# carlobaldassi/GaussDCA.jl

Measured on AMD Instinct MI355X. Metric: end-to-end gDCA sec + achieved Cholesky TFLOP/s, N=500 M=50k q=21, higher is better.
Workload: dtype f64

## Files before the change

### gaussdca.jl_amd/csrc/gdca_api.hip

```cpp
#include <algorithm>
#include <ctype.h>
#include <math.h>
#include <stdio.h>
#include <stdlib.h>
#include <string.h>
#include <strings.h>

#include "gdca_internal.h"
#include "gdca_launch.h"

#define MAX_EV 1024
#define N_SCRATCH 10

struct gdca_buf {
    void *p;
    size_t cap;
};

struct gdca_gate {
    hipEvent_t ev[4];
    int next, last, armed, refs;
    hipStream_t batch_stream;
};

// ... 246 lines not shown
    if (!strncasecmp(key, "GDCA_", 5)) key += 5;
    for (; key[n] && n + 1 < sizeof(k); ++n) k[n] = (char)toupper((unsigned char)key[n]);
    k[n] = 0;
    if (!strcmp(k, "SWEEP_TRACE")) {
        if (strlen(value) >= sizeof(t->sweep_trace)) return false;
        strcpy(t->sweep_trace, value);
        return true;
    }
    if (!strcmp(k, "HAMMING_MODE")) {
        const char c = (char)tolower((unsigned char)value[0]);
        t->hamming_mode = c == 'f' ? 0 : (c == 'b' ? 1 : (c == 'm' ? 2 : -1));
        return c == 'f' || c == 'b' || c == 'm' || c == 'a' || c == 0;
    }
    if (!strcmp(k, "FORCE_FALLBACK")) {
        t->force_fallback = (*value && strcmp(value, "0") != 0) ? 1 : 0;
        return true;
    }
    long x = 0;
    if (strcmp(k, "REFINE") && strcmp(k, "REFINE_COND") && !parse_long(value, &x)) return false;
    struct { const char *name; int *field; long lo, hi; } ints[] = {
        {"GROUP", &t->group, -1, 4},        {"RAMP", &t->ramp, 0, 1},          {"RAGGED", &t->ragged, 0, 1},
        {"REM_TAIL", &t->rem_tail, -1, 1 << 20}, {"PANEL_HALVES", &t->panel_halves, -1, 1}, {"SLAB", &t->slab, 0, 1},
        {"RING", &t->ring, 2, 8},           {"MCUS", &t->mcus, -1, 32},        {"MCU_SOLO", &t->mcu_solo, -1, 1},       {"SWEEP_DEBUG", &t->sweep_debug, 0, 63}, {"SWEEP_RETRIES", &t->sweep_retries, 0, 5},
        {"TALLY_TJ", &t->tally_tj, 0, 32},  {"TALLY_SKIP", &t->tally_skip, 0, 1}, {"MERGE", &t->merge, 1, 8},        {"MERGE_BLOCKS", &t->merge_blocks, 1, 64},
        {"MERGE_MCUS", &t->merge_mcus, -1, 16},  {"MERGE_GROUP", &t->merge_group, -1, 4}, {"MERGE_TILES", &t->merge_tiles, 1, 1 << 20},
        {"CHOLESKY", &t->cholesky, 0, 2},  {"PHASED_FRONTS", &t->phased_fronts, 0, 1}, {"PHASED_GRIDS", &t->phased_grids, -1, 8}, {"PHASED_STREAMS", &t->phased_streams, 1, 64},
        {"ENERGY_CHUNK", &t->energy_chunk, 0, 1 << 30}, {"PAIR_CHUNK", &t->pair_chunk, 0, 1 << 30},
    };
    for (auto &e : ints)
        if (!strcmp(k, e.name)) {
            if (x < e.lo || x > e.hi) return false;
            *e.field = (int)x;
            return true;
        }
    if (!strcmp(k, "REFINE")) {
        const char c = (char)tolower((unsigned char)value[0]);
        if (c == 'a' || !strcmp(value, "-1")) t->refine = -1;
        else if (!strcmp(value, "0") || !strcasecmp(value, "off") || c == 'n') t->refine = 0;
        else if (!strcmp(value, "1") || !strcasecmp(value, "on") || c == 'y') t->refine = 1;
        else return false;
        return true;
    }
    if (!strcmp(k, "REFINE_COND")) {
        char *end = nullptr;
        const double x = strtod(value, &end);
        if (end == value || *end || !(x > 0.0)) return false;
        t->refine_cond = x;
// ... 1 lines not shown
    }
    if (!strcmp(k, "SWEEP_TIMEOUT_MS")) {
        if (x < 0) return false;
        t->sweep_timeout_ms = x;
        return true;
    }
    return false;
}

void gdca_tuning_from_env(gdca_tuning *t)
{
    memset(t, 0, sizeof(*t));
    t->group = -1;
    t->ramp = 1;
    t->ragged = 1;
    t->rem_tail = -1;
    t->panel_halves = -1;
    t->slab = 1;
    t->ring = 8;
    t->mcus = -1;
    t->mcu_solo = -1;
    t->sweep_retries = 2;
    t->tally_skip = 1;
    t->hamming_mode = -1;
    t->merge = 8;
    t->merge_blocks = 57;
    t->merge_mcus = -1;
    t->merge_group = -1;
    t->merge_tiles = 2300;
    t->phased_fronts = 1;
    t->phased_grids = -1;
    t->phased_streams = 4;
    t->refine = -1;
    t->refine_cond = 1e6;
    t->cholesky = 1;
    static const char *const names[] = {"GDCA_GROUP", "GDCA_RAMP", "GDCA_RAGGED", "GDCA_REM_TAIL", "GDCA_PANEL_HALVES", "GDCA_SLAB",
                                        "GDCA_RING", "GDCA_MCUS", "GDCA_SWEEP_DEBUG", "GDCA_SWEEP_TIMEOUT_MS", "GDCA_SWEEP_RETRIES", "GDCA_TALLY_TJ", "GDCA_TALLY_SKIP",
                                        "GDCA_HAMMING_MODE", "GDCA_FORCE_FALLBACK", "GDCA_MERGE", "GDCA_MERGE_BLOCKS",
                                        "GDCA_MERGE_MCUS", "GDCA_MERGE_GROUP", "GDCA_MERGE_TILES", "GDCA_REFINE", "GDCA_REFINE_COND", "GDCA_CHOLESKY", "GDCA_SWEEP_TRACE", "GDCA_PHASED_FRONTS", "GDCA_PHASED_GRIDS", "GDCA_PHASED_STREAMS", "GDCA_MCU_SOLO", "GDCA_ENERGY_CHUNK", "GDCA_PAIR_CHUNK"};
    for (const char *nm : names)
        if (const char *v = getenv(nm)) (void)gdca_tuning_set(t, nm, v);
}

static gdca_status fail(gdca_ctx *ctx, gdca_status st, const char *fmt, const char *a, const char *b)
{
    if (ctx) snprintf(ctx->err, sizeof(ctx->err), fmt, a, b);
    return st;
}

#define HIPCHK(expr)                                                                      \
    do {                                                                                  \
        hipError_t e_ = (expr);                                                           \
        if (e_ != hipSuccess) return fail(ctx, GDCA_EHIP, "%s: %s", #expr, hipGetErrorString(e_)); \
    } while (0)

#define CHK(expr)                         \
    do {                                  \
        gdca_status s_ = (expr);          \
        if (s_ != GDCA_OK) return s_;     \
    } while (0)

static gdca_status ensure(gdca_ctx *ctx, gdca_buf &b, size_t bytes)
{
    if (bytes == 0) bytes = 16;
    if (b.cap >= bytes) return GDCA_OK;
    if (b.p) {
        HIPCHK(hipStreamSynchronize(ctx->stream));
        HIPCHK(hipFree(b.p));
        b.p = nullptr;
        b.cap = 0;
    }
    const size_t want = (bytes + 255) & ~(size_t)255;
    hipError_t e = hipMalloc(&b.p, want);
// ... 248 lines not shown
        memcpy(lead->err, msg, sizeof(msg));
    }
    return st;
}

static gdca_status upload_done(gdca_ctx *ctx)
{
    HIPCHK(hipEventRecord(ctx->ev_upload, ctx->stream));
    HIPCHK(hipEventSynchronize(ctx->ev_upload));
    return GDCA_OK;
}

static double inverse_flops_model(double n)
{
    return (n * n * n / 3.0 + n * n / 2.0 + n / 6.0) + (2.0 * n * n * n / 3.0 + n * n / 2.0 + 5.0 * n / 6.0);
}

static int round_up(int x, int m)
{
    return (x + m - 1) / m * m;
}

static gdca_status weights_stage(gdca_ctx *ctx, const int8_t *Zd, int N, int M, int q, double theta_in, int fixed_thresh,
                                 bool want_theta_only, int mark_after_theta)
{
    hipStream_t s = ctx->stream;
    gdca_dev_scalars *sc = (gdca_dev_scalars *)ctx->sc.p;
    CHK(ensure(ctx, ctx->hist, (size_t)N * 32 * sizeof(uint32_t)));
    if (fixed_thresh >= 0) {
        gdca_launch_set_thresh(s, sc, fixed_thresh);
    } else {
        if (theta_in < 0.0) {
            gdca_fill_async(s, ctx->hist.p, 0, (size_t)N * 32 * sizeof(uint32_t));
            gdca_launch_column_hist(s, Zd, (uint32_t *)ctx->hist.p, N, M);
        }
        gdca_launch_theta_finalize(s, (const uint32_t *)ctx->hist.p, N, M, theta_in, sc);
    }
    CHK(check_launch(ctx, "theta"));
    if (mark_after_theta >= 0) CHK(mark(ctx, mark_after_theta));
    if (want_theta_only) return GDCA_OK;

    const int Mt = (M + GDCA_HTILE - 1) / GDCA_HTILE;
    CHK(ensure(ctx, ctx->Zb, gdca_bitplane_bytes(N, M)));
    CHK(ensure(ctx, ctx->hcnt, (size_t)Mt * GDCA_HTILE * sizeof(int32_t)));
    if (!ctx->tune.force_fallback && ctx->tune.hamming_mode != 0) CHK(ensure(ctx, ctx->hcand, gdca_hamming_cand_cap(M) * 8));
    const bool fp4 = !ctx->tune.force_fallback && ctx->tune.hamming_mode == 2;
    if (fp4) CHK(ensure(ctx, ctx->himg, gdca_fp4_image_bytes(N, M)));
    CHK(ensure(ctx, ctx->nk, (size_t)M * sizeof(int32_t)));
    CHK(ensure(ctx, ctx->W, (size_t)M * sizeof(double)));
    CHK(ensure(ctx, ctx->Wfix, (size_t)M * sizeof(unsigned long long)));
    gdca_fill_async(s, ctx->hcnt.p, 0, (size_t)Mt * GDCA_HTILE * sizeof(int32_t));
    gdca_launch_bitplane_pack(s, Zd, (uint32_t *)ctx->Zb.p, N, M, q, sc);
    if (ctx->tune.force_fallback)
        gdca_launch_hamming_fallback(s, Zd, (int32_t *)ctx->hcnt.p, N, M, sc);
    else
        gdca_launch_hamming(s, (const uint32_t *)ctx->Zb.p, Zd, (int32_t *)ctx->hcnt.p, N, M, sc, ctx->tune.hamming_mode, ctx->hcand.p, fp4 ? ctx->himg.p : nullptr);
    gdca_launch_weights(s, (const int32_t *)ctx->hcnt.p, M, gdca_fix_shift(M), (int32_t *)ctx->nk.p,
                        (double *)ctx->W.p, (unsigned long long *)ctx->Wfix.p);
    gdca_launch_meff(s, (const double *)ctx->W.p, M, sc);
    return check_launch(ctx, "weights");
}

static bool norm1_settled(const gdca_ctx *ctx, int N, int q, double pc)
{
    const double pi_cap = (1.0 - pc) + pc / (double)q;
    return pc > 0.0 && 2.0 * (double)N * pi_cap * (double)q * (double)q / pc <= ctx->tune.refine_cond && ctx->tune.refine != 1;
}

static gdca_status tally_stage(gdca_ctx *ctx, const int8_t *Zd, int N, int M, int q, const double *Meff_dev, double pc,
                               int mode, double *Pi_true_out, double *out, size_t ld, bool want_norm1 = false)
{
    hipStream_t s = ctx->stream;
    const int sdim = q - 1, n = N * sdim;
    const int shift = gdca_fix_shift(M);
    const int TJ = gdca_tally_tj(q, ctx->tune.tally_tj);
    const bool skip = gdca_tally_skip(q, TJ, ctx->tune.tally_skip, M);
    const size_t keep_list = (size_t)N * M * sizeof(uint32_t);
    if (skip) CHK(ensure(ctx, ctx->keep, keep_list + (size_t)N * sizeof(int) + N));
    CHK(ensure(ctx, ctx->Zt, (size_t)N * M));
    CHK(ensure(ctx, ctx->Zp, (size_t)round_up(N, 64) * M + 64));
    CHK(ensure(ctx, ctx->Pifix, (size_t)N * 32 * sizeof(unsigned long long)));
    CHK(ensure(ctx, ctx->Pipc, (size_t)n * sizeof(double)));
    gdca_launch_transpose_i8(s, Zd, (int8_t *)ctx->Zt.p, N, M);
    gdca_launch_colblock(s, Zd, (int8_t *)ctx->Zp.p, N, M, TJ);
    gdca_fill_async(s, ctx->Pifix.p, 0, (size_t)N * 32 * sizeof(unsigned long long));
    gdca_launch_pi_tally(s, Zd, (const unsigned long long *)ctx->Wfix.p, (unsigned long long *)ctx->Pifix.p, N, M, q,
                         (gdca_dev_scalars *)ctx->sc.p);
    gdca_launch_pi_finalize(s, (const unsigned long long *)ctx->Pifix.p, N, q, shift, Meff_dev, pc, Pi_true_out,
                            (double *)ctx->Pipc.p, want_norm1 ? &((gdca_dev_scalars *)ctx->sc.p)->pi_max : nullptr);
    const bool tm = want_norm1 && ctx->timing && ctx->n_ev >= 18;
    if (tm) CHK(mark(ctx, 9));
    uint32_t *keep = skip ? (uint32_t *)ctx->keep.p : nullptr;
    int *keep_n = skip ? (int *)((char *)ctx->keep.p + keep_list) : nullptr;
    uint8_t *sigma = skip ? (uint8_t *)(keep_n + N) : nullptr;
    if (skip)
        gdca_launch_tally_keep(s, (const int8_t *)ctx->Zt.p, (const unsigned long long *)ctx->Pifix.p, keep, keep_n, sigma, N, M, q);
    gdca_launch_pair_tally(s, (const int8_t *)ctx->Zp.p, (const int8_t *)ctx->Zt.p,
                           (const unsigned long long *)ctx->Wfix.p, N, M, q, shift, Meff_dev, pc,
                           (const double *)ctx->Pipc.p, mode, out, ld, TJ, keep, keep_n, sigma,
                           (const unsigned long long *)ctx->Pifix.p);
    if (tm) CHK(mark(ctx, 10));
    if (want_norm1 && !norm1_settled(ctx, N, q, pc))
        gdca_launch_cov_norm1(s, out, ld, N, q, pc, ctx->tune.refine_cond, (gdca_dev_scalars *)ctx->sc.p, ctx->tune.refine == 1);
    return check_launch(ctx, "tally");
}

static gdca_status inverse_job(gdca_ctx *ctx, int n, int n_pad, gdca_inverse_job *job)
{
    const size_t pbytes = (size_t)n_pad * GDCA_TILE * sizeof(double);
    const int nblk = n_pad / GDCA_TILE;
    const size_t sg = (size_t)4 * GDCA_TILE * 4 * GDCA_TILE * sizeof(double);
    const size_t fbytes = gdca_inverse_flag_bytes(n_pad);
    CHK(ensure(ctx, ctx->G, (size_t)8 * pbytes));
    CHK(ensure(ctx, ctx->H, (size_t)8 * pbytes));
    CHK(ensure(ctx, ctx->P, (size_t)GDCA_TILE * GDCA_TILE * sizeof(double)));
    CHK(ensure(ctx, ctx->Sg, 4 * sg + fbytes + (size_t)3 * (nblk + 2) * sizeof(int)));
    if (ctx->item0_cap < 3 * (nblk + 2)) {
        if (ctx->item0_host) HIPCHK(hipHostFree(ctx->item0_host));
// ... 408 lines not shown
    r.q = q;
    r.n = N * (q - 1);
    r.n_pad = round_up(r.n, GDCA_TILE);
    r.Z = Z_dev;
    r.pij = pij;
    r.p = *p;
    r.timed = timed;
    r.stamped = ctx->stamped;
    r.front_batch = r.score_batch = 1;
    r.tally_timed = timed && !pij && ctx->tune.refine != 0;
    r.fn_timed = false;
}

static gdca_status run_front(gdca_ctx *ctx, const int8_t *Z_dev, int32_t N, int32_t M, int32_t q, const gdca_params *p)
{
    CHK(begin(ctx));
    hipStream_t s = ctx->stream;
    const int sdim = q - 1, n = N * sdim, n_pad = round_up(n, GDCA_TILE);
    const bool timed = ctx->timing;
    if (timed) CHK(need_events(ctx, 18));
    gdca_dev_scalars *sc = (gdca_dev_scalars *)ctx->sc.p;

    if (timed) CHK(mark(ctx, 0));
    CHK(weights_stage(ctx, Z_dev, N, M, q, p->theta, -1, false, timed ? 1 : -1));
    if (timed) CHK(mark(ctx, 2));

    CHK(ensure(ctx, ctx->A, (size_t)n_pad * n_pad * sizeof(double)));
    CHK(tally_stage(ctx, Z_dev, N, M, q, &sc->Meff, p->pseudocount, 1, nullptr, (double *)ctx->A.p, (size_t)n_pad, ctx->tune.refine != 0));
    gdca_launch_pad_identity(s, (double *)ctx->A.p, n, n_pad);
    if (p->score == GDCA_SCORE_DI) {
        CHK(ensure(ctx, ctx->Dblk, (size_t)N * sdim * sdim * sizeof(double)));
        CHK(ensure(ctx, ctx->Ld, (size_t)N * sdim * sdim * sizeof(double)));
        gdca_launch_save_diag_blocks(s, (const double *)ctx->A.p, (size_t)n_pad, N, sdim, (double *)ctx->Dblk.p);
        gdca_launch_diag_chol(s, (const double *)ctx->Dblk.p, N, sdim, (double *)ctx->Ld.p);
    }
    CHK(check_launch(ctx, "covariance"));
    if (timed) CHK(mark(ctx, 3));
    pending_front(ctx, Z_dev, N, M, q, p, nullptr, timed);
    return GDCA_OK;
}

static gdca_status run_inverse(gdca_ctx *ctx)
{
    hipStream_t s = ctx->stream;
    const bool timed = ctx->pend.timed;
    hipEvent_t *ev = ctx->ev;
    int n_upd = 0;
    double upd_flops = 0.0;
    if (ctx->gate) HIPCHK(gate_wait(ctx->gate, s));
    if (timed) HIPCHK(hipEventRecord(ev[6], s));
    CHK(inverse_stage(ctx, ctx->pend.n, ctx->pend.n_pad, timed, &n_upd, &upd_flops));
// ... 477 lines not shown
    double *sv;
    CHK(ranking_stage(ctx, S_dev, ctx->pend.N, rk->sep, rk->len, &ii, &jj, &sv));
    const size_t at = (size_t)k * (size_t)rk->len;
    return ranking_to_host(ctx, rk->len, ii, jj, sv, rk->i_out + at, rk->j_out + at, rk->score_out + at);
}

static gdca_status run_multi(gdca_ctx *ctx, const int8_t *Z_dev, int N, int M, int q, const gdca_params *p, int K, double *S_dev, size_t S_stride,
                             gdca_stats *st, const multi_rank *rk)
{
    hipStream_t s = ctx->stream;
    const int sdim = q - 1, n = N * sdim, n_pad = round_up(n, GDCA_TILE);
    gdca_status mst[GDCA_MULTI_MAX];
    bool done[GDCA_MULTI_MAX];
    for (int k = 0; k < K; ++k) {
        memset(&st[k], 0, sizeof(st[k]));
        mst[k] = GDCA_OK;
        done[k] = false;
    }
    CHK(begin(ctx));
    const bool timed = ctx->timing;
    if (timed) CHK(need_events(ctx, 18));
    gdca_dev_scalars *sc = (gdca_dev_scalars *)ctx->sc.p;
    if (timed) CHK(mark(ctx, 0));
    CHK(weights_stage(ctx, Z_dev, N, M, q, p[0].theta, -1, false, timed ? 1 : -1));
    if (timed) CHK(mark(ctx, 2));
    CHK(ensure(ctx, ctx->Pij, (size_t)n * n * sizeof(double)));
    CHK(ensure(ctx, ctx->A, (size_t)n_pad * n_pad * sizeof(double)));
    CHK(ensure(ctx, ctx->sc_front, sizeof(gdca_dev_scalars)));
    CHK(tally_stage(ctx, Z_dev, N, M, q, &sc->Meff, p[0].pseudocount, 0, nullptr, (double *)ctx->Pij.p, (size_t)n));
    HIPCHK(hipMemcpyAsync(ctx->sc_front.p, sc, sizeof(gdca_dev_scalars), hipMemcpyDeviceToDevice, s));
    pending_front(ctx, Z_dev, N, M, q, &p[0], (const double *)ctx->Pij.p, timed);
    double ms_theta = 0.0, ms_weights = 0.0;
    bool first = true;
    for (int k0 = 0; k0 < K; ++k0) {
        if (done[k0]) continue;
        const double pc = p[k0].pseudocount;
        bool di = false;
        for (int k = k0; k < K; ++k) di = di || (p[k].pseudocount == pc && p[k].score == GDCA_SCORE_DI);
        if (!first) {
            HIPCHK(hipMemcpyAsync(sc, ctx->sc_front.p, sizeof(gdca_dev_scalars), hipMemcpyDeviceToDevice, s));
            ctx->pend.at = gdca_pending::progress{};
            if (timed) CHK(mark(ctx, 2));
        }
        ctx->pend.p = p[k0];
        ctx->pend.fn_timed = false;
        CHK(cov_from_pij_stage(ctx, N, M, q, pc, (double *)ctx->A.p, (size_t)n_pad, ctx->tune.refine != 0));
        gdca_launch_pad_identity(s, (double *)ctx->A.p, n, n_pad);
        if (di) {
            CHK(ensure(ctx, ctx->Dblk, (size_t)N * sdim * sdim * sizeof(double)));
            CHK(ensure(ctx, ctx->Ld, (size_t)N * sdim * sdim * sizeof(double)));
            gdca_launch_save_diag_blocks(s, (const double *)ctx->A.p, (size_t)n_pad, N, sdim, (double *)ctx->Dblk.p);
            gdca_launch_diag_chol(s, (const double *)ctx->Dblk.p, N, sdim, (double *)ctx->Ld.p);
// ... 835 lines not shown
```

### gaussdca.jl_amd/csrc/gdca_internal.h

```cpp
#pragma once

#include <hip/hip_runtime.h>
#include <stdint.h>

#include "gdca.h"

#define GDCA_TILE 128
#define GDCA_HTILE 128
#define GDCA_MAXQ 31
#define GDCA_STAMPS 20

struct gdca_dev_scalars {
    double theta;
    double Meff;
    unsigned long long pair_sum;
    int thresh;
    int info;
    int bad_symbol;
    int di_noconv;
    int ham_mode;
    int ham_cand;
    unsigned long long ham_ncand;
    unsigned long long sweep_cycles, sweep_ticks;
    double inv_norm1;
    double ns_resid;
    double mat_norm1;
    double pi_max;
    unsigned long long stamp[GDCA_STAMPS];
    int ham_cand2;
    int pad_;
};

struct gdca_tuning {
    int group;
    int ramp;
    int ragged;
    int rem_tail;
    int panel_halves;
    int slab;
    int ring;
    int mcus;
    int mcu_solo;
    int sweep_debug;
    long sweep_timeout_ms;
    int sweep_retries;
    int tally_tj;
    int tally_skip;
    int hamming_mode;
    int force_fallback;
    int merge;
    int merge_blocks;
    int merge_mcus;
    int merge_group;
    int merge_tiles;
    int phased_fronts;
    int phased_grids;
    int phased_streams;
    int refine;
    double refine_cond;
    int cholesky;
    int energy_chunk;
    int pair_chunk;
    char sweep_trace[256];
};
void gdca_tuning_from_env(gdca_tuning *t);
bool gdca_tuning_set(gdca_tuning *t, const char *key, const char *value);

void gdca_launch_transpose_i8(hipStream_t s, const int8_t *Z, int8_t *Zt, int N, int M);
void gdca_launch_column_hist(hipStream_t s, const int8_t *Z, uint32_t *cnt, int N, int M);
void gdca_launch_theta_finalize(hipStream_t s, const uint32_t *cnt, int N, int M, double theta_in,
                                gdca_dev_scalars *sc);
void gdca_launch_set_thresh(hipStream_t s, gdca_dev_scalars *sc, int thresh);

size_t gdca_bitplane_bytes(int N, int M);
void gdca_launch_bitplane_pack(hipStream_t s, const int8_t *Z, uint32_t *Zb, int N, int M, int q,
                               gdca_dev_scalars *sc);
size_t gdca_hamming_cand_cap(int M);
size_t gdca_fp4_image_bytes(int N, int M);
void gdca_launch_hamming_fp4_probe(hipStream_t s, const uint32_t *Zb, int N, int M, int nprobe, gdca_dev_scalars *sc);
void gdca_launch_hamming_fp4(hipStream_t s, const uint32_t *Zb, void *img, int N, int M, gdca_dev_scalars *sc, void *cand_list, unsigned cap);
void gdca_launch_hamming(hipStream_t s, const uint32_t *Zb, const int8_t *Z, int32_t *cnt, int N, int M, gdca_dev_scalars *sc, int force,
                         void *cand_list, void *fp4_img);
void gdca_launch_hamming_fallback(hipStream_t s, const int8_t *Z, int32_t *cnt, int N, int M, const gdca_dev_scalars *sc);
void gdca_launch_weights(hipStream_t s, const int32_t *cnt, int M, int fix_shift, int32_t *n_out, double *W,
                         unsigned long long *Wfix);
void gdca_launch_meff(hipStream_t s, const double *W, int M, gdca_dev_scalars *sc);
void gdca_launch_fix_weights(hipStream_t s, const double *W, int M, int fix_shift, unsigned long long *Wfix,
                             gdca_dev_scalars *sc);
int gdca_fix_shift(int M);

void gdca_launch_pi_tally(hipStream_t s, const int8_t *Z, const unsigned long long *Wfix,
                          unsigned long long *Pifix, int N, int M, int q, gdca_dev_scalars *sc);
void gdca_launch_pi_finalize(hipStream_t s, const unsigned long long *Pifix, int N, int q, int fix_shift,
                             const double *Meff_dev, double pc, double *Pi_true, double *Pi_pc, double *pi_max = nullptr);
void gdca_launch_cov_norm1(hipStream_t s, const double *C, size_t ld, int N, int q, double pc, double cond_limit, gdca_dev_scalars *sc,
                           int always);
int gdca_tally_tj(int q, int tj_wanted);
void gdca_launch_colblock(hipStream_t s, const int8_t *Z, int8_t *Zc, int N, int M, int TJ);
bool gdca_tally_skip(int q, int TJ, int skip_wanted, int M);
void gdca_launch_tally_keep(hipStream_t s, const int8_t *Zt, const unsigned long long *Pifix, uint32_t *keep, int *keep_n,
                            uint8_t *sigma, int N, int M, int q);
void gdca_launch_pair_tally(hipStream_t s, const int8_t *Zc, const int8_t *Zt, const unsigned long long *Wfix,
                            int N, int M, int q, int fix_shift, const double *Meff_dev, double pc,
                            const double *Pi_pc, int mode, double *out, size_t ld, int TJ, const uint32_t *keep = nullptr,
                            const int *keep_n = nullptr, const uint8_t *sigma = nullptr, const unsigned long long *Pifix = nullptr);
void gdca_launch_cov_from_pij(hipStream_t s, const double *Pij, const double *Pi_pc, int N, int q, double pc, double *out, size_t ld);

void gdca_launch_add_pseudocount(hipStream_t s, const double *Pi_true, const double *Pij_true, int N, int q,
                                 double pc, double *Pi, double *Pij);
void gdca_launch_covariance(hipStream_t s, const double *Pi, const double *Pij, int n, double *C);
void gdca_launch_pad_identity(hipStream_t s, double *A, int n, int n_pad);
void gdca_launch_copy_in(hipStream_t s, const double *src, int n, double *dst, int n_pad);
void gdca_launch_copy_in_neg(hipStream_t s, const double *src, int n, double *dst, int n_pad);
void gdca_launch_copy_out_neg_sym(hipStream_t s, const double *A, int n_pad, double *dst, int n);
void gdca_launch_publish_scalars(hipStream_t s, const gdca_dev_scalars *sc, gdca_dev_scalars *host_mapped);
void gdca_launch_save_diag_blocks(hipStream_t s, const double *C, size_t ld, int N, int sdim, double *D);

struct gdca_inverse_ws {
    double *G[8];
    double *H[8];
    double *P;
    double *Sg[2];
    double *Pg[2];
    unsigned *flags;
// ... 63 lines not shown
```

### gaussdca.jl_amd/csrc/k_tally.hip

```cpp
#include "gdca_internal.h"
#include "gdca_launch.h"
#include <cstdlib>

typedef unsigned long long u64;

struct k_pi_tally_args {
    const int8_t *Z;
    const u64 *Wfix;
    u64 *Pifix;
    int N;
    int M;
    int seq_per_block;
    int q;
    gdca_dev_scalars *sc;
};
static inline k_pi_tally_args k_pi_tally_mk(const int8_t *Z, const u64 *Wfix, u64 *Pifix, int N, int M, int seq_per_block, int q, gdca_dev_scalars *sc)
{
    return k_pi_tally_args{Z, Wfix, Pifix, N, M, seq_per_block, q, sc};
}
template <int CAP>
__global__ __launch_bounds__(128) void k_pi_tally(const BatchArgs<k_pi_tally_args, CAP> B_)
{
    GDCA_MEMBER(B_);
    const int8_t *__restrict__ Z = a_.Z;
// ... 189 lines not shown
        const int k = k0 + r * 4 + ty, c = c0 + tx;
        tile[r * 4 + ty][tx] = (k < M && c < N) ? Z[(size_t)k * N + c] : (int8_t)0;
    }
    __syncthreads();
    const int nb = 64 / TJ;
    for (int e = threadIdx.x; e < 64 * 64; e += 256) {
        const int blk = e / (64 * TJ), rem = e % (64 * TJ);
        const int kl = rem / TJ, cl = rem % TJ;
        const int k = k0 + kl;
        const int cb = c0 / TJ + blk;
        if (blk < nb && k < M && cb * TJ < ((N + TJ - 1) / TJ) * TJ)
            Zc[((size_t)cb * M + k) * TJ + cl] = tile[kl][blk * TJ + cl];
    }
}

void gdca_launch_colblock(hipStream_t s, const int8_t *Z, int8_t *Zc, int N, int M, int TJ)
{
    dim3 grid((N + 63) / 64, (M + 63) / 64);
    (gdca_launch<k_colblock_args, k_colblock<1>, k_colblock<GDCA_MAXB>>(grid, dim3(256), 0, s, k_colblock_mk(Z, Zc, N, M, TJ)));
}

#define KEEP_THREADS 256
#define KEEP_SLABS 16
struct k_tally_keep_args {
    const int8_t *Zt;
    const u64 *Pifix;
    uint32_t *keep;
    int *keep_n;
    uint8_t *sigma;
    int N;
    int M;
    int q;
};
static inline k_tally_keep_args k_tally_keep_mk(const int8_t *Zt, const u64 *Pifix, uint32_t *keep, int *keep_n, uint8_t *sigma, int N, int M, int q)
{
    return k_tally_keep_args{Zt, Pifix, keep, keep_n, sigma, N, M, q};
}
template <int CAP>
__global__ __launch_bounds__(KEEP_THREADS) void k_tally_keep(const BatchArgs<k_tally_keep_args, CAP> B_)
{
    GDCA_MEMBER(B_);
    const int8_t *__restrict__ Zt = a_.Zt;
    const u64 *__restrict__ Pifix = a_.Pifix;
    uint32_t *__restrict__ keep = a_.keep;
    int M = a_.M;
    int q = a_.q;
    constexpr int NW = KEEP_THREADS / 64;
    __shared__ unsigned wcnt[KEEP_SLABS * NW], woff[KEEP_SLABS * NW];
    const int i = blockIdx.x;
    const int t = threadIdx.x, lane = t & 63, wv = t >> 6;
    const u64 *P = Pifix + (size_t)i * 32;
    unsigned sig = 1;
    u64 best = P[1];
    for (int a = 2; a <= q; ++a) {
        const u64 v = P[a];
        if (v > best) {
            best = v;
            sig = (unsigned)a;
        }
    }
    const int8_t *zi = Zt + (size_t)i * M;
    uint32_t *out = keep + (size_t)i * M;
    const u64 lt = (1ull << lane) - 1ull;
    unsigned base = 0;
    for (int kc = 0; kc < M; kc += KEEP_THREADS * KEEP_SLABS) {
        unsigned raw[KEEP_SLABS], pos[KEEP_SLABS];
#pragma unroll
        for (int u = 0; u < KEEP_SLABS; ++u) {
            const int k = kc + u * KEEP_THREADS + t;
            raw[u] = k < M ? (unsigned)(uint8_t)zi[k] : 0u;
        }
#pragma unroll
        for (int u = 0; u < KEEP_SLABS; ++u) {
            const bool kp = (raw[u] - 1u) < (unsigned)q && raw[u] != sig;
            const u64 bal = __ballot(kp);
            pos[u] = kp ? (unsigned)__popcll(bal & lt) : ~0u;
            if (lane == 0) wcnt[u * NW + wv] = (unsigned)__popcll(bal);
        }
        __syncthreads();
        if (t < KEEP_SLABS * NW) {
            unsigned o = base;
            for (int e = 0; e < t; ++e) o += wcnt[e];
            woff[t] = o;
        }
        __syncthreads();
#pragma unroll
        for (int u = 0; u < KEEP_SLABS; ++u)
            if (pos[u] != ~0u) out[woff[u * NW + wv] + pos[u]] = ((unsigned)(kc + u * KEEP_THREADS + t) << 5) | raw[u];
        base = woff[KEEP_SLABS * NW - 1] + wcnt[KEEP_SLABS * NW - 1];
        __syncthreads();
    }
    if (t == 0) {
        a_.keep_n[i] = (int)base;
        a_.sigma[i] = (uint8_t)sig;
    }
}

void gdca_launch_tally_keep(hipStream_t s, const int8_t *Zt, const u64 *Pifix, uint32_t *keep, int *keep_n, uint8_t *sigma, int N, int M, int q)
{
    (gdca_launch<k_tally_keep_args, k_tally_keep<1>, k_tally_keep<GDCA_MAXB>>(dim3(N), dim3(KEEP_THREADS), 0, s, k_tally_keep_mk(Zt, Pifix, keep, keep_n, sigma, N, M, q)));
}

struct k_pair_tally_args {
    const int8_t *Zc;
    const int8_t *Zt;
    const u64 *Wfix;
    int N;
    int M;
    int q;
    int fix_shift;
    const double *Meff_dev;
    double pc;
    const double *Pi_pc;
    int mode;
    double *out;
    size_t ld;
    const uint32_t *keep;
    const int *keep_n;
    const uint8_t *sigma;
    const u64 *Pifix;
};
static inline k_pair_tally_args k_pair_tally_mk(const int8_t *Zc, const int8_t *Zt, const u64 *Wfix, int N, int M, int q, int fix_shift, const double *Meff_dev, double pc, const double *Pi_pc, int mode, double *out, size_t ld,
                                                const uint32_t *keep, const int *keep_n, const uint8_t *sigma, const u64 *Pifix)
// ... 259 lines not shown
```

### gaussdca.jl_amd/csrc/k_theta.hip

```cpp
#include "gdca_internal.h"
#include "gdca_launch.h"

struct k_transpose_i8_args {
    const int8_t *Z;
    int8_t *Zt;
    int N;
    int M;
};
static inline k_transpose_i8_args k_transpose_i8_mk(const int8_t *Z, int8_t *Zt, int N, int M)
{
    return k_transpose_i8_args{Z, Zt, N, M};
}
template <int CAP>
__global__ __launch_bounds__(256) void k_transpose_i8(const BatchArgs<k_transpose_i8_args, CAP> B_)
{
    GDCA_MEMBER(B_);
    const int8_t *__restrict__ Z = a_.Z;
    int8_t *__restrict__ Zt = a_.Zt;
    int N = a_.N;
    int M = a_.M;
    __shared__ int8_t tile[64][65];
    const int k0 = blockIdx.y * 64, i0 = blockIdx.x * 64;
    const int tx = threadIdx.x & 63, ty = threadIdx.x >> 6;
#pragma unroll
// ... 53 lines not shown
            for (int u = 0; u < 16; ++u) h[z[u]][t] += 1;
            p += (size_t)16 * N;
        }
        for (; k < kend; ++k) {
            h[p[0] & 31][t] += 1;
            p += N;
        }
#pragma unroll
        for (int z = 0; z < 32; ++z) {
            const uint32_t v = h[z][t];
            if (v) atomicAdd(&cnt[(size_t)i * 32 + z], v);
        }
    }
}

void gdca_launch_column_hist(hipStream_t s, const int8_t *Z, uint32_t *cnt, int N, int M)
{
    const int cb = (N + 255) / 256;
    int chunks = (256 + cb - 1) / cb;
    int spb = (M + chunks - 1) / chunks;
    if (spb < 64) spb = 64;
    chunks = (M + spb - 1) / spb;
    (gdca_launch<k_column_hist_args, k_column_hist<1>, k_column_hist<GDCA_MAXB>>(dim3(cb, chunks), dim3(256), 0, s, k_column_hist_mk(Z, cnt, N, M, spb)));
}

struct k_theta_finalize_args {
    const uint32_t *cnt;
    int N;
    int M;
    double theta_in;
    gdca_dev_scalars *sc;
};
static inline k_theta_finalize_args k_theta_finalize_mk(const uint32_t *cnt, int N, int M, double theta_in, gdca_dev_scalars *sc)
{
    return k_theta_finalize_args{cnt, N, M, theta_in, sc};
}
template <int CAP>
__global__ __launch_bounds__(256) void k_theta_finalize(const BatchArgs<k_theta_finalize_args, CAP> B_)
{
    GDCA_MEMBER(B_);
    const uint32_t *__restrict__ cnt = a_.cnt;
    int N = a_.N;
    int M = a_.M;
    double theta_in = a_.theta_in;
    gdca_dev_scalars *sc = a_.sc;
    __shared__ unsigned long long red[256];
// ... 62 lines not shown
```

Measured before the change: 47.36.

## Fuse front-end passes over Z into a single prepare kernel and merge pi tally with keep

Adds a k_prepare kernel that reads the alignment once per tile and in the same pass produces the bitplane pack, the transposed Zt, the column-blocked Zc, the column histogram and the symbol validity check. These were previously separate kernels that each read Z again. Also adds a k_pi_keep kernel that computes the single-site tally from Zt and builds the keep list in the same block, replacing the separate pi_tally and tally_keep launches. Both paths are on by default through a new FRONT_FUSED knob; the cost is a more complex kernel with heavy shared-memory use and possible changes in occupancy.

Result: no change. 47.72 (median of 6 runs) (+0.8%).

```diff
diff --git a/gaussdca.jl_amd/csrc/gdca_api.hip b/gaussdca.jl_amd/csrc/gdca_api.hip
--- a/gaussdca.jl_amd/csrc/gdca_api.hip
+++ b/gaussdca.jl_amd/csrc/gdca_api.hip
@@ -292,7 +292,7 @@
         {"GROUP", &t->group, -1, 4},        {"RAMP", &t->ramp, 0, 1},          {"RAGGED", &t->ragged, 0, 1},
         {"REM_TAIL", &t->rem_tail, -1, 1 << 20}, {"PANEL_HALVES", &t->panel_halves, -1, 1}, {"SLAB", &t->slab, 0, 1},
         {"RING", &t->ring, 2, 8},           {"MCUS", &t->mcus, -1, 32},        {"MCU_SOLO", &t->mcu_solo, -1, 1},       {"SWEEP_DEBUG", &t->sweep_debug, 0, 63}, {"SWEEP_RETRIES", &t->sweep_retries, 0, 5},
-        {"TALLY_TJ", &t->tally_tj, 0, 32},  {"TALLY_SKIP", &t->tally_skip, 0, 1}, {"MERGE", &t->merge, 1, 8},        {"MERGE_BLOCKS", &t->merge_blocks, 1, 64},
+        {"TALLY_TJ", &t->tally_tj, 0, 32},  {"TALLY_SKIP", &t->tally_skip, 0, 1}, {"FRONT_FUSED", &t->front_fused, 0, 1}, {"MERGE", &t->merge, 1, 8},        {"MERGE_BLOCKS", &t->merge_blocks, 1, 64},
         {"MERGE_MCUS", &t->merge_mcus, -1, 16},  {"MERGE_GROUP", &t->merge_group, -1, 4}, {"MERGE_TILES", &t->merge_tiles, 1, 1 << 20},
         {"CHOLESKY", &t->cholesky, 0, 2},  {"PHASED_FRONTS", &t->phased_fronts, 0, 1}, {"PHASED_GRIDS", &t->phased_grids, -1, 8}, {"PHASED_STREAMS", &t->phased_streams, 1, 64},
         {"ENERGY_CHUNK", &t->energy_chunk, 0, 1 << 30}, {"PAIR_CHUNK", &t->pair_chunk, 0, 1 << 30},
@@ -340,6 +340,7 @@
     t->mcu_solo = -1;
     t->sweep_retries = 2;
     t->tally_skip = 1;
+    t->front_fused = 1;
     t->hamming_mode = -1;
     t->merge = 8;
     t->merge_blocks = 57;
@@ -353,7 +354,7 @@
     t->refine_cond = 1e6;
     t->cholesky = 1;
     static const char *const names[] = {"GDCA_GROUP", "GDCA_RAMP", "GDCA_RAGGED", "GDCA_REM_TAIL", "GDCA_PANEL_HALVES", "GDCA_SLAB",
-                                        "GDCA_RING", "GDCA_MCUS", "GDCA_SWEEP_DEBUG", "GDCA_SWEEP_TIMEOUT_MS", "GDCA_SWEEP_RETRIES", "GDCA_TALLY_TJ", "GDCA_TALLY_SKIP",
+                                        "GDCA_RING", "GDCA_MCUS", "GDCA_SWEEP_DEBUG", "GDCA_SWEEP_TIMEOUT_MS", "GDCA_SWEEP_RETRIES", "GDCA_TALLY_TJ", "GDCA_TALLY_SKIP", "GDCA_FRONT_FUSED",
                                         "GDCA_HAMMING_MODE", "GDCA_FORCE_FALLBACK", "GDCA_MERGE", "GDCA_MERGE_BLOCKS",
                                         "GDCA_MERGE_MCUS", "GDCA_MERGE_GROUP", "GDCA_MERGE_TILES", "GDCA_REFINE", "GDCA_REFINE_COND", "GDCA_CHOLESKY", "GDCA_SWEEP_TRACE", "GDCA_PHASED_FRONTS", "GDCA_PHASED_GRIDS", "GDCA_PHASED_STREAMS", "GDCA_MCU_SOLO", "GDCA_ENERGY_CHUNK", "GDCA_PAIR_CHUNK"};
     for (const char *nm : names)
@@ -366,7 +367,12 @@
     return st;
 }
 
-#define HIPCHK(expr)                                                                      \
+static gdca_status fail(gdca_ctx *ctx, gdca_status st, const char *msg)
+{
+    return fail(ctx, st, "%s%s", msg, "");
+}
+
+#define HIPCHK(expr)                                                                     \
     do {                                                                                  \
         hipError_t e_ = (expr);                                                           \
         if (e_ != hipSuccess) return fail(ctx, GDCA_EHIP, "%s: %s", #expr, hipGetErrorString(e_)); \
@@ -661,12 +667,21 @@
 }
 
 static gdca_status weights_stage(gdca_ctx *ctx, const int8_t *Zd, int N, int M, int q, double theta_in, int fixed_thresh,
-                                 bool want_theta_only, int mark_after_theta)
+                                 bool want_theta_only, int mark_after_theta, bool fused = false)
 {
     hipStream_t s = ctx->stream;
     gdca_dev_scalars *sc = (gdca_dev_scalars *)ctx->sc.p;
+    if (fused && (fixed_thresh >= 0 || want_theta_only)) return fail(ctx, GDCA_EINVAL, "weights_stage: the fused form takes theta and runs the whole stage");
     CHK(ensure(ctx, ctx->hist, (size_t)N * 32 * sizeof(uint32_t)));
-    if (fixed_thresh >= 0) {
+    if (fused) {
+        CHK(ensure(ctx, ctx->Zb, gdca_bitplane_bytes(N, M)));
+        CHK(ensure(ctx, ctx->Zt, (size_t)N * M));
+        CHK(ensure(ctx, ctx->Zp, (size_t)round_up(N, 64) * M + 64));
+        if (theta_in < 0.0) gdca_fill_async(s, ctx->hist.p, 0, (size_t)N * 32 * sizeof(uint32_t));
+        gdca_launch_prepare(s, Zd, (uint32_t *)ctx->Zb.p, (int8_t *)ctx->Zt.p, (int8_t *)ctx->Zp.p, theta_in < 0.0 ? (uint32_t *)ctx->hist.p : nullptr,
+                            N, M, q, gdca_tally_tj(q, ctx->tune.tally_tj), sc);
+        gdca_launch_theta_finalize(s, (const uint32_t *)ctx->hist.p, N, M, theta_in, sc);
+    } else if (fixed_thresh >= 0) {
         gdca_launch_set_thresh(s, sc, fixed_thresh);
     } else {
         if (theta_in < 0.0) {
@@ -689,7 +704,7 @@
     CHK(ensure(ctx, ctx->W, (size_t)M * sizeof(double)));
     CHK(ensure(ctx, ctx->Wfix, (size_t)M * sizeof(unsigned long long)));
     gdca_fill_async(s, ctx->hcnt.p, 0, (size_t)Mt * GDCA_HTILE * sizeof(int32_t));
-    gdca_launch_bitplane_pack(s, Zd, (uint32_t *)ctx->Zb.p, N, M, q, sc);
+    if (!fused) gdca_launch_bitplane_pack(s, Zd, (uint32_t *)ctx->Zb.p, N, M, q, sc);
     if (ctx->tune.force_fallback)
         gdca_launch_hamming_fallback(s, Zd, (int32_t *)ctx->hcnt.p, N, M, sc);
     else
@@ -707,7 +722,7 @@
 }
 
 static gdca_status tally_stage(gdca_ctx *ctx, const int8_t *Zd, int N, int M, int q, const double *Meff_dev, double pc,
-                               int mode, double *Pi_true_out, double *out, size_t ld, bool want_norm1 = false)
+                               int mode, double *Pi_true_out, double *out, size_t ld, bool want_norm1 = false, bool fused = false)
 {
     hipStream_t s = ctx->stream;
     const int sdim = q - 1, n = N * sdim;
@@ -720,19 +735,27 @@
     CHK(ensure(ctx, ctx->Zp, (size_t)round_up(N, 64) * M + 64));
     CHK(ensure(ctx, ctx->Pifix, (size_t)N * 32 * sizeof(unsigned long long)));
     CHK(ensure(ctx, ctx->Pipc, (size_t)n * sizeof(double)));
-    gdca_launch_transpose_i8(s, Zd, (int8_t *)ctx->Zt.p, N, M);
-    gdca_launch_colblock(s, Zd, (int8_t *)ctx->Zp.p, N, M, TJ);
-    gdca_fill_async(s, ctx->Pifix.p, 0, (size_t)N * 32 * sizeof(unsigned long long));
-    gdca_launch_pi_tally(s, Zd, (const unsigned long long *)ctx->Wfix.p, (unsigned long long *)ctx->Pifix.p, N, M, q,
-                         (gdca_dev_scalars *)ctx->sc.p);
+    uint32_t *keep = skip ? (uint32_t *)ctx->keep.p : nullptr;
+    int *keep_n = skip ? (int *)((char *)ctx->keep.p + keep_list) : nullptr;
+    uint8_t *sigma = skip ? (uint8_t *)(keep_n + N) : nullptr;
+    const bool pi_keep = fused && skip && gdca_pi_keep_fused(N, M);
+    if (!fused) {
+        gdca_launch_transpose_i8(s, Zd, (int8_t *)ctx->Zt.p, N, M);
+        gdca_launch_colblock(s, Zd, (int8_t *)ctx->Zp.p, N, M, TJ);
+    }
+    if (pi_keep) {
+        gdca_launch_pi_keep(s, (const int8_t *)ctx->Zt.p, (const unsigned long long *)ctx->Wfix.p, (unsigned long long *)ctx->Pifix.p, keep, keep_n, sigma,
+                            N, M, q, (gdca_dev_scalars *)ctx->sc.p);
+    } else {
+        gdca_fill_async(s, ctx->Pifix.p, 0, (size_t)N * 32 * sizeof(unsigned long long));
+        gdca_launch_pi_tally(s, Zd, (const unsigned long long *)ctx->Wfix.p, (unsigned long long *)ctx->Pifix.p, N, M, q,
+                             (gdca_dev_scalars *)ctx->sc.p);
+    }
     gdca_launch_pi_finalize(s, (const unsigned long long *)ctx->Pifix.p, N, q, shift, Meff_dev, pc, Pi_true_out,
                             (double *)ctx->Pipc.p, want_norm1 ? &((gdca_dev_scalars *)ctx->sc.p)->pi_max : nullptr);
     const bool tm = want_norm1 && ctx->timing && ctx->n_ev >= 18;
     if (tm) CHK(mark(ctx, 9));
-    uint32_t *keep = skip ? (uint32_t *)ctx->keep.p : nullptr;
-    int *keep_n = skip ? (int *)((char *)ctx->keep.p + keep_list) : nullptr;
-    uint8_t *sigma = skip ? (uint8_t *)(keep_n + N) : nullptr;
-    if (skip)
+    if (skip && !pi_keep)
         gdca_launch_tally_keep(s, (const int8_t *)ctx->Zt.p, (const unsigned long long *)ctx->Pifix.p, keep, keep_n, sigma, N, M, q);
     gdca_launch_pair_tally(s, (const int8_t *)ctx->Zp.p, (const int8_t *)ctx->Zt.p,
                            (const unsigned long long *)ctx->Wfix.p, N, M, q, shift, Meff_dev, pc,
@@ -1187,11 +1210,12 @@
     gdca_dev_scalars *sc = (gdca_dev_scalars *)ctx->sc.p;
 
     if (timed) CHK(mark(ctx, 0));
-    CHK(weights_stage(ctx, Z_dev, N, M, q, p->theta, -1, false, timed ? 1 : -1));
+    const bool fused = ctx->tune.front_fused != 0;
+    CHK(weights_stage(ctx, Z_dev, N, M, q, p->theta, -1, false, timed ? 1 : -1, fused));
     if (timed) CHK(mark(ctx, 2));
 
     CHK(ensure(ctx, ctx->A, (size_t)n_pad * n_pad * sizeof(double)));
-    CHK(tally_stage(ctx, Z_dev, N, M, q, &sc->Meff, p->pseudocount, 1, nullptr, (double *)ctx->A.p, (size_t)n_pad, ctx->tune.refine != 0));
+    CHK(tally_stage(ctx, Z_dev, N, M, q, &sc->Meff, p->pseudocount, 1, nullptr, (double *)ctx->A.p, (size_t)n_pad, ctx->tune.refine != 0, fused));
     gdca_launch_pad_identity(s, (double *)ctx->A.p, n, n_pad);
     if (p->score == GDCA_SCORE_DI) {
         CHK(ensure(ctx, ctx->Dblk, (size_t)N * sdim * sdim * sizeof(double)));
@@ -1715,12 +1739,13 @@
     if (timed) CHK(need_events(ctx, 18));
     gdca_dev_scalars *sc = (gdca_dev_scalars *)ctx->sc.p;
     if (timed) CHK(mark(ctx, 0));
-    CHK(weights_stage(ctx, Z_dev, N, M, q, p[0].theta, -1, false, timed ? 1 : -1));
+    const bool fused = ctx->tune.front_fused != 0;
+    CHK(weights_stage(ctx, Z_dev, N, M, q, p[0].theta, -1, false, timed ? 1 : -1, fused));
     if (timed) CHK(mark(ctx, 2));
     CHK(ensure(ctx, ctx->Pij, (size_t)n * n * sizeof(double)));
     CHK(ensure(ctx, ctx->A, (size_t)n_pad * n_pad * sizeof(double)));
     CHK(ensure(ctx, ctx->sc_front, sizeof(gdca_dev_scalars)));
-    CHK(tally_stage(ctx, Z_dev, N, M, q, &sc->Meff, p[0].pseudocount, 0, nullptr, (double *)ctx->Pij.p, (size_t)n));
+    CHK(tally_stage(ctx, Z_dev, N, M, q, &sc->Meff, p[0].pseudocount, 0, nullptr, (double *)ctx->Pij.p, (size_t)n, false, fused));
     HIPCHK(hipMemcpyAsync(ctx->sc_front.p, sc, sizeof(gdca_dev_scalars), hipMemcpyDeviceToDevice, s));
     pending_front(ctx, Z_dev, N, M, q, &p[0], (const double *)ctx->Pij.p, timed);
     double ms_theta = 0.0, ms_weights = 0.0;
diff --git a/gaussdca.jl_amd/csrc/gdca_internal.h b/gaussdca.jl_amd/csrc/gdca_internal.h
--- a/gaussdca.jl_amd/csrc/gdca_internal.h
+++ b/gaussdca.jl_amd/csrc/gdca_internal.h
@@ -46,6 +46,7 @@
     int sweep_retries;
     int tally_tj;
     int tally_skip;
+    int front_fused;
     int hamming_mode;
     int force_fallback;
     int merge;
@@ -68,6 +69,8 @@
 
 void gdca_launch_transpose_i8(hipStream_t s, const int8_t *Z, int8_t *Zt, int N, int M);
 void gdca_launch_column_hist(hipStream_t s, const int8_t *Z, uint32_t *cnt, int N, int M);
+void gdca_launch_prepare(hipStream_t s, const int8_t *Z, uint32_t *Zb, int8_t *Zt, int8_t *Zc, uint32_t *cnt, int N, int M, int q, int TJ,
+                         gdca_dev_scalars *sc);
 void gdca_launch_theta_finalize(hipStream_t s, const uint32_t *cnt, int N, int M, double theta_in,
                                 gdca_dev_scalars *sc);
 void gdca_launch_set_thresh(hipStream_t s, gdca_dev_scalars *sc, int thresh);
@@ -100,6 +103,9 @@
 bool gdca_tally_skip(int q, int TJ, int skip_wanted, int M);
 void gdca_launch_tally_keep(hipStream_t s, const int8_t *Zt, const unsigned long long *Pifix, uint32_t *keep, int *keep_n,
                             uint8_t *sigma, int N, int M, int q);
+bool gdca_pi_keep_fused(int N, int M);
+void gdca_launch_pi_keep(hipStream_t s, const int8_t *Zt, const unsigned long long *Wfix, unsigned long long *Pifix, uint32_t *keep, int *keep_n,
+                         uint8_t *sigma, int N, int M, int q, gdca_dev_scalars *sc);
 void gdca_launch_pair_tally(hipStream_t s, const int8_t *Zc, const int8_t *Zt, const unsigned long long *Wfix,
                             int N, int M, int q, int fix_shift, const double *Meff_dev, double pc,
                             const double *Pi_pc, int mode, double *out, size_t ld, int TJ, const uint32_t *keep = nullptr,
diff --git a/gaussdca.jl_amd/csrc/k_tally.hip b/gaussdca.jl_amd/csrc/k_tally.hip
--- a/gaussdca.jl_amd/csrc/k_tally.hip
+++ b/gaussdca.jl_amd/csrc/k_tally.hip
@@ -235,6 +235,42 @@
 
 #define KEEP_THREADS 256
 #define KEEP_SLABS 16
+__device__ __forceinline__ unsigned keep_list(const int8_t *__restrict__ zi, uint32_t *__restrict__ out, int M, int q, unsigned sig, unsigned *wcnt, unsigned *woff)
+{
+    constexpr int NW = KEEP_THREADS / 64;
+    const int t = threadIdx.x, lane = t & 63, wv = t >> 6;
+    const u64 lt = (1ull << lane) - 1ull;
+    unsigned base = 0;
+    for (int kc = 0; kc < M; kc += KEEP_THREADS * KEEP_SLABS) {
+        unsigned raw[KEEP_SLABS], pos[KEEP_SLABS];
+#pragma unroll
+        for (int u = 0; u < KEEP_SLABS; ++u) {
+            const int k = kc + u * KEEP_THREADS + t;
+            raw[u] = k < M ? (unsigned)(uint8_t)zi[k] : 0u;
+        }
+#pragma unroll
+        for (int u = 0; u < KEEP_SLABS; ++u) {
+            const bool kp = (raw[u] - 1u) < (unsigned)q && raw[u] != sig;
+            const u64 bal = __ballot(kp);
+            pos[u] = kp ? (unsigned)__popcll(bal & lt) : ~0u;
+            if (lane == 0) wcnt[u * NW + wv] = (unsigned)__popcll(bal);
+        }
+        __syncthreads();
+        if (t < KEEP_SLABS * NW) {
+            unsigned o = base;
+            for (int e = 0; e < t; ++e) o += wcnt[e];
+            woff[t] = o;
+        }
+        __syncthreads();
+#pragma unroll
+        for (int u = 0; u < KEEP_SLABS; ++u)
+            if (pos[u] != ~0u) out[woff[u * NW + wv] + pos[u]] = ((unsigned)(kc + u * KEEP_THREADS + t) << 5) | raw[u];
+        base = woff[KEEP_SLABS * NW - 1] + wcnt[KEEP_SLABS * NW - 1];
+        __syncthreads();
+    }
+    return base;
+}
+
 struct k_tally_keep_args {
     const int8_t *Zt;
     const u64 *Pifix;
@@ -261,7 +297,7 @@
     constexpr int NW = KEEP_THREADS / 64;
     __shared__ unsigned wcnt[KEEP_SLABS * NW], woff[KEEP_SLABS * NW];
     const int i = blockIdx.x;
-    const int t = threadIdx.x, lane = t & 63, wv = t >> 6;
+    const int t = threadIdx.x;
     const u64 *P = Pifix + (size_t)i * 32;
     unsigned sig = 1;
     u64 best = P[1];
@@ -274,35 +310,7 @@
     }
     const int8_t *zi = Zt + (size_t)i * M;
     uint32_t *out = keep + (size_t)i * M;
-    const u64 lt = (1ull << lane) - 1ull;
-    unsigned base = 0;
-    for (int kc = 0; kc < M; kc += KEEP_THREADS * KEEP_SLABS) {
-        unsigned raw[KEEP_SLABS], pos[KEEP_SLABS];
-#pragma unroll
-        for (int u = 0; u < KEEP_SLABS; ++u) {
-            const int k = kc + u * KEEP_THREADS + t;
-            raw[u] = k < M ? (unsigned)(uint8_t)zi[k] : 0u;
-        }
-#pragma unroll
-        for (int u = 0; u < KEEP_SLABS; ++u) {
-            const bool kp = (raw[u] - 1u) < (unsigned)q && raw[u] != sig;
-            const u64 bal = __ballot(kp);
-            pos[u] = kp ? (unsigned)__popcll(bal & lt) : ~0u;
-            if (lane == 0) wcnt[u * NW + wv] = (unsigned)__popcll(bal);
-        }
-        __syncthreads();
-        if (t < KEEP_SLABS * NW) {
-            unsigned o = base;
-            for (int e = 0; e < t; ++e) o += wcnt[e];
-            woff[t] = o;
-        }
-        __syncthreads();
-#pragma unroll
-        for (int u = 0; u < KEEP_SLABS; ++u)
-            if (pos[u] != ~0u) out[woff[u * NW + wv] + pos[u]] = ((unsigned)(kc + u * KEEP_THREADS + t) << 5) | raw[u];
-        base = woff[KEEP_SLABS * NW - 1] + wcnt[KEEP_SLABS * NW - 1];
-        __syncthreads();
-    }
+    const unsigned base = keep_list(zi, out, M, q, sig, wcnt, woff);
     if (t == 0) {
         a_.keep_n[i] = (int)base;
         a_.sigma[i] = (uint8_t)sig;
@@ -312,6 +320,98 @@
 void gdca_launch_tally_keep(hipStream_t s, const int8_t *Zt, const u64 *Pifix, uint32_t *keep, int *keep_n, uint8_t *sigma, int N, int M, int q)
 {
     (gdca_launch<k_tally_keep_args, k_tally_keep<1>, k_tally_keep<GDCA_MAXB>>(dim3(N), dim3(KEEP_THREADS), 0, s, k_tally_keep_mk(Zt, Pifix, keep, keep_n, sigma, N, M, q)));
+}
+
+struct k_pi_keep_args {
+    const int8_t *Zt;
+    const u64 *Wfix;
+    u64 *Pifix;
+    uint32_t *keep;
+    int *keep_n;
+    uint8_t *sigma;
+    gdca_dev_scalars *sc;
+    int N;
+    int M;
+    int q;
+};
+static inline k_pi_keep_args k_pi_keep_mk(const int8_t *Zt, const u64 *Wfix, u64 *Pifix, uint32_t *keep, int *keep_n, uint8_t *sigma, gdca_dev_scalars *sc, int N, int M, int q)
+{
+    return k_pi_keep_args{Zt, Wfix, Pifix, keep, keep_n, sigma, sc, N, M, q};
+}
+template <int CAP>
+__global__ __launch_bounds__(KEEP_THREADS) void k_pi_keep(const BatchArgs<k_pi_keep_args, CAP> B_)
+{
+    GDCA_MEMBER(B_);
+    const int8_t *__restrict__ Zt = a_.Zt;
+    const u64 *__restrict__ Wfix = a_.Wfix;
+    uint32_t *__restrict__ keep = a_.keep;
+    int M = a_.M;
+    int q = a_.q;
+    constexpr int NW = KEEP_THREADS / 64;
+    extern __shared__ u64 h[];
+    __shared__ u64 P[32];
+    __shared__ unsigned wcnt[KEEP_SLABS * NW], woff[KEEP_SLABS * NW];
+    const int i = blockIdx.x;
+    const int t = threadIdx.x, lane = t & 63, wv = t >> 6;
+    const int8_t *zi = Zt + (size_t)i * M;
+#pragma unroll
+    for (int z = 0; z < 32; ++z) h[z * KEEP_THREADS + t] = 0;
+    unsigned bad = 0;
+    for (int kc = 0; kc < M; kc += KEEP_THREADS * KEEP_SLABS) {
+        unsigned raw[KEEP_SLABS];
+        u64 w[KEEP_SLABS];
+#pragma unroll
+        for (int u = 0; u < KEEP_SLABS; ++u) {
+            const int k = kc + u * KEEP_THREADS + t;
+            raw[u] = k < M ? (unsigned)(uint8_t)zi[k] : 1u;
+            w[u] = k < M ? Wfix[k] : 0ull;
+        }
+#pragma unroll
+        for (int u = 0; u < KEEP_SLABS; ++u) {
+            bad |= (raw[u] - 1u) >= (unsigned)q;
+            h[(raw[u] & 31) * KEEP_THREADS + t] += w[u];
+        }
+    }
+    if (bad) atomicOr(&a_.sc->bad_symbol, 1);
+    __syncthreads();
+    for (int z = wv * (32 / NW); z < (wv + 1) * (32 / NW); ++z) {
+        u64 v = 0;
+#pragma unroll
+        for (int j = 0; j < NW; ++j) v += h[z * KEEP_THREADS + lane + 64 * j];
+#pragma unroll
+        for (int o = 32; o > 0; o >>= 1) v += __shfl_xor(v, o, 64);
+        if (lane == 0) {
+            P[z] = v;
+            a_.Pifix[(size_t)i * 32 + z] = v;
+        }
+    }
+    __syncthreads();
+    unsigned sig = 1;
+    u64 best = P[1];
+    for (int a = 2; a <= q; ++a) {
+        const u64 v = P[a];
+        if (v > best) {
+            best = v;
+            sig = (unsigned)a;
+        }
+    }
+    uint32_t *out = keep + (size_t)i * M;
+    const unsigned base = keep_list(zi, out, M, q, sig, wcnt, woff);
+    if (t == 0) {
+        a_.keep_n[i] = (int)base;
+        a_.sigma[i] = (uint8_t)sig;
+    }
+}
+
+bool gdca_pi_keep_fused(int N, int M)
+{
+    return N >= 32 || M <= (1 << 16);
+}
+
+void gdca_launch_pi_keep(hipStream_t s, const int8_t *Zt, const u64 *Wfix, u64 *Pifix, uint32_t *keep, int *keep_n, uint8_t *sigma, int N, int M, int q,
+                         gdca_dev_scalars *sc)
+{
+    (gdca_launch<k_pi_keep_args, k_pi_keep<1>, k_pi_keep<GDCA_MAXB>>(dim3(N), dim3(KEEP_THREADS), 32 * KEEP_THREADS * sizeof(u64), s, k_pi_keep_mk(Zt, Wfix, Pifix, keep, keep_n, sigma, sc, N, M, q)));
 }
 
 struct k_pair_tally_args {
diff --git a/gaussdca.jl_amd/csrc/k_theta.hip b/gaussdca.jl_amd/csrc/k_theta.hip
--- a/gaussdca.jl_amd/csrc/k_theta.hip
+++ b/gaussdca.jl_amd/csrc/k_theta.hip
@@ -99,6 +99,176 @@
     if (spb < 64) spb = 64;
     chunks = (M + spb - 1) / spb;
     (gdca_launch<k_column_hist_args, k_column_hist<1>, k_column_hist<GDCA_MAXB>>(dim3(cb, chunks), dim3(256), 0, s, k_column_hist_mk(Z, cnt, N, M, spb)));
+}
+
+#define PREP_COLS 64
+#define PREP_LDW 17
+struct k_prepare_args {
+    const int8_t *Z;
+    uint32_t *Zb;
+    int8_t *Zt;
+    int8_t *Zc;
+    uint32_t *cnt;
+    gdca_dev_scalars *sc;
+    int N;
+    int M;
+    int NW;
+    int q;
+    int TJ;
+};
+static inline k_prepare_args k_prepare_mk(const int8_t *Z, uint32_t *Zb, int8_t *Zt, int8_t *Zc, uint32_t *cnt, gdca_dev_scalars *sc, int N, int M, int NW, int q, int TJ)
+{
+    return k_prepare_args{Z, Zb, Zt, Zc, cnt, sc, N, M, NW, q, TJ};
+}
+template <int CAP>
+__global__ __launch_bounds__(256) void k_prepare(const BatchArgs<k_prepare_args, CAP> B_)
+{
+    GDCA_MEMBER(B_);
+    const int8_t *__restrict__ Z = a_.Z;
+    uint32_t *__restrict__ Zb = a_.Zb;
+    int8_t *__restrict__ Zt = a_.Zt;
+    int8_t *__restrict__ Zc = a_.Zc;
+    uint32_t *__restrict__ cnt = a_.cnt;
+    gdca_dev_scalars *sc = a_.sc;
+    const int N = a_.N, M = a_.M, NW = a_.NW, q = a_.q, TJ = a_.TJ;
+    __shared__ uint32_t tile[GDCA_HTILE * PREP_LDW];
+    __shared__ uint32_t h[32 * PREP_COLS];
+    const uint8_t *tile8 = reinterpret_cast<const uint8_t *>(tile);
+    const int t = threadIdx.x;
+    const int c0 = blockIdx.x * PREP_COLS;
+    const int Mt = (M + GDCA_HTILE - 1) / GDCA_HTILE;
+    const bool zfast = (N & 3) == 0 && (reinterpret_cast<uintptr_t>(Z) & 3) == 0;
+    const bool tfast = (M & 3) == 0;
+    const uint32_t over = (0x7fu - (uint32_t)q) * 0x01010101u;
+    uint32_t bad = 0;
+    if (cnt)
+        for (int e = t; e < 32 * PREP_COLS; e += 256) h[e] = 0;
+
+    uint32_t d[8];
+    auto fetch = [&](int tl) {
+        if (zfast) {
+#pragma unroll
+            for (int r = 0; r < 8; ++r) {
+                const int e = t + 256 * r;
+                const int k = tl * GDCA_HTILE + (e >> 4), c = c0 + 4 * (e & 15);
+                d[r] = (k < M && c < N) ? *reinterpret_cast<const uint32_t *>(Z + (size_t)k * N + c) : 0x01010101u;
+            }
+#pragma unroll
+            for (int r = 0; r < 8; ++r) {
+                const uint32_t v = d[r];
+                bad |= (v - 0x01010101u) & ~v & 0x80808080u;
+                bad |= (((v & 0x7f7f7f7fu) + over) | v) & 0x80808080u;
+                const int e = t + 256 * r;
+                if (!(tl * GDCA_HTILE + (e >> 4) < M && c0 + 4 * (e & 15) < N)) d[r] = 0;
+            }
+        } else {
+#pragma unroll
+            for (int r = 0; r < 8; ++r) {
+                const int e = t + 256 * r;
+                const int k = tl * GDCA_HTILE + (e >> 4), c = c0 + 4 * (e & 15);
+                uint32_t v = 0;
+                if (k < M && c < N) {
+                    const int8_t *src = Z + (size_t)k * N + c;
+                    const int nb = min(4, N - c);
+#pragma unroll 1
+                    for (int j = 0; j < nb; ++j) {
+                        const uint32_t raw = (uint32_t)(uint8_t)src[j];
+                        bad |= (raw - 1u) >= (uint32_t)q;
+                        v |= raw << (8 * j);
+                    }
+                }
+                d[r] = v;
+            }
+        }
+    };
+
+    int tl = blockIdx.y;
+    if (tl < Mt) fetch(tl);
+    for (; tl < Mt; tl += gridDim.y) {
+        const int k0 = tl * GDCA_HTILE;
+        const int rows = min(GDCA_HTILE, M - k0);
+        __syncthreads();
+#pragma unroll
+        for (int r = 0; r < 8; ++r) {
+            const int e = t + 256 * r;
+            tile[(e >> 4) * PREP_LDW + (e & 15)] = d[r];
+        }
+        __syncthreads();
+        if (tl + (int)gridDim.y < Mt) fetch(tl + (int)gridDim.y);
+
+        {
+            const int kl = t & (GDCA_HTILE - 1), w = t >> 7, wg = c0 / 32 + w;
+            if (wg < NW) {
+                uint32_t pl[5] = {0, 0, 0, 0, 0};
+#pragma unroll
+                for (int j = 0; j < 8; ++j) {
+                    const uint32_t v = tile[kl * PREP_LDW + w * 8 + j];
+#pragma unroll
+                    for (int p = 0; p < 5; ++p) {
+                        const uint32_t b = (v >> p) & 0x01010101u;
+                        pl[p] |= (((b * 0x01020408u) >> 24) & 0xFu) << (4 * j);
+                    }
+                }
+#pragma unroll
+                for (int p = 0; p < 5; ++p) Zb[(((size_t)tl * 5 + p) * NW + wg) * GDCA_HTILE + kl] = pl[p];
+            }
+        }
+        {
+            const int lj = TJ == 32 ? 3 : 2;
+            const int NBJ = (N + TJ - 1) / TJ;
+            uint32_t *Zc4 = reinterpret_cast<uint32_t *>(Zc);
+#pragma unroll
+            for (int r = 0; r < 8; ++r) {
+                const int e = t + 256 * r;
+                const int blk = e >> (7 + lj), rem = e & ((GDCA_HTILE << lj) - 1);
+                const int kl = rem >> lj, cw = rem & ((1 << lj) - 1);
+                const int cb = c0 / TJ + blk;
+                if (kl < rows && cb < NBJ) Zc4[((((size_t)cb * M + k0 + kl) * TJ) >> 2) + cw] = tile[kl * PREP_LDW + (blk << lj) + cw];
+            }
+        }
+        if (tfast) {
+            uint32_t *Zt4 = reinterpret_cast<uint32_t *>(Zt);
+#pragma unroll
+            for (int r = 0; r < 8; ++r) {
+                const int e = t + 256 * r;
+                const int kk = (e & 15) + 16 * ((e >> 6) & 1), c = ((e >> 4) & 3) + 4 * (e >> 7);
+                const uint8_t *b = tile8 + (size_t)(4 * kk) * (4 * PREP_LDW) + c;
+                const uint32_t v = (uint32_t)b[0] | ((uint32_t)b[4 * PREP_LDW] << 8) | ((uint32_t)b[8 * PREP_LDW] << 16) | ((uint32_t)b[12 * PREP_LDW] << 24);
+                if (c0 + c < N && 4 * kk < rows) Zt4[(((size_t)(c0 + c) * M + k0) >> 2) + kk] = v;
+            }
+        } else {
+#pragma unroll 4
+            for (int r = 0; r < 32; ++r) {
+                const int e = t + 256 * r;
+                const int kl = e & (GDCA_HTILE - 1), c = e >> 7;
+                if (c0 + c < N && kl < rows) Zt[(size_t)(c0 + c) * M + k0 + kl] = (int8_t)tile8[kl * (4 * PREP_LDW) + c];
+            }
+        }
+        if (cnt) {
+            const int c = t & 63;
+            for (int kl = t >> 6; kl < rows; kl += 4) atomicAdd(&h[(tile8[kl * (4 * PREP_LDW) + c] & 31) * PREP_COLS + c], 1u);
+        }
+    }
+    if (bad) atomicOr(&sc->bad_symbol, 1);
+    if (cnt) {
+        __syncthreads();
+#pragma unroll
+        for (int r = 0; r < 8; ++r) {
+            const int e = t + 256 * r;
+            const int c = e >> 5, z = e & 31;
+            const uint32_t v = h[z * PREP_COLS + c];
+            if (v && c0 + c < N) atomicAdd(&cnt[(size_t)(c0 + c) * 32 + z], v);
+        }
+    }
+}
+
+void gdca_launch_prepare(hipStream_t s, const int8_t *Z, uint32_t *Zb, int8_t *Zt, int8_t *Zc, uint32_t *cnt, int N, int M, int q, int TJ,
+                         gdca_dev_scalars *sc)
+{
+    const int strips = (N + PREP_COLS - 1) / PREP_COLS, Mt = (M + GDCA_HTILE - 1) / GDCA_HTILE, NW = (N + 31) / 32;
+    int gy = (768 + strips - 1) / strips;
+    if (gy > Mt) gy = Mt;
+    (gdca_launch<k_prepare_args, k_prepare<1>, k_prepare<GDCA_MAXB>>(dim3(strips, gy), dim3(256), 0, s, k_prepare_mk(Z, Zb, Zt, Zc, cnt, sc, N, M, NW, q, TJ)));
 }
 
 struct k_theta_finalize_args {
```
